# fverdoja/Fast-3D-Pointcloud-Segmentation

Measured on AMD Instinct MI355X. Metric: Mpoints/sec segmented end-to-end, 1M-pt RGB-D frames, higher is better.
Workload: dtype f32

## Files before the change

### fast-3d-pointcloud-segmentation_amd/csrc/f3ds_hip.hip

```cpp
#include <hip/hip_runtime.h>

#include <algorithm>
#include <cmath>
#include <atomic>
#include <map>
#include <chrono>
#include <cstdio>
#include <cstdlib>
#include <cstring>
#include <string>
#include <type_traits>
#include <mutex>
#include <set>
#include <vector>

#include "../../include/f3ds.h"
#include "f3ds_algo.h"
#include "f3ds_glasbey.h"
#include "f3ds_eval.h"
#include "f3ds_dev.h"
#include "f3ds_levels.h"
#include "f3ds_eval_levels.h"
#include "f3ds_rgbd.h"
#include "f3ds_label_image.h"
// ... 492 lines not shown
    const uint32_t capV = (uint32_t)std::max<uint64_t>(256u, std::min<uint64_t>(fin, dcap));
    c->vox_cap = capV;
    uint64_t *k0, *k1; uint32_t *ploc, *v0, *v1, *part, *vkey, *vcount, *seg_start, *list; uint2* bo_te; float* vf; int* pt_voxel;
    const uint32_t nchunks = (dcap + DS_CHUNK - 1u) / DS_CHUNK;
    ENSURE(c->pslot, n, ploc); ENSURE(c->keys0, dcap, k0); ENSURE(c->keys1, dcap, k1); ENSURE(c->vals0, dcap, v0); ENSURE(c->vals1, dcap, v1);
    { uint32_t* w; ENSURE(c->hcnt, (size_t)ntiles * VT_TAB * 2 + 2u * nchunks, w); bo_te = reinterpret_cast<uint2*>(w); part = w + (size_t)ntiles * VT_TAB * 2; }
    ENSURE(c->vkey, (size_t)capV * 3, vkey); ENSURE(c->vcount, capV, vcount); ENSURE(c->vf, (size_t)capV * 12, vf);
    ENSURE(c->seg_start, (size_t)capV + 1, seg_start); ENSURE(c->vlist, n, list); ENSURE(c->pt_voxel, n, pt_voxel);
    { uint32_t *f, *incl; ENSURE(c->flags, capV, f); ENSURE(c->incl, capV, incl); }
    c->idxbits = -1; c->ks = nullptr; c->vs = nullptr;
    rec<d_tile_keys>(c, std::min<uint32_t>(ntiles, (uint32_t)g_grid_cap * 16u), 0u, c->d_pts, n, c->fa, c->d_grid, ploc, k0, v0, dcap, tile_bits, c->d_dc);
    uint64_t* ks; uint32_t* vs;
    int rc = radix_sort(c, k0, v0, k1, v1, dcap, code_bits + tile_bits, &ks, &vs, VT_CNT_BITS, &c->d_dc->seg_count);
    if (rc) return rc;
    rec<d_desc_part>(c, nchunks, 0u, ks, dcap, tile_bits, part, c->d_dc);
    rec<d_desc_offsets>(c, 1u, 0u, part, dcap, capV, seg_start, c->d_dc);
    rec<d_desc_apply>(c, nchunks, 0u, ks, vs, dcap, capV, tile_bits, c->fa, c->d_grid, part, bo_te, seg_start, vkey, c->d_dc);
    rec<d_tile_place>(c, std::min<uint32_t>(ntiles, (uint32_t)g_grid_cap * 16u), 0u, ploc, n, bo_te, list, pt_voxel, c->d_dc);
    rec<d_voxel_list_accum>(c, std::min<uint32_t>(grid_wide(capV, 256), std::max<uint32_t>(64u, grid_wide(n / 8u, 256))), 0u, c->d_pts, list, seg_start, c->fa, vf, vcount, c->d_dc, capV);
    c->vox_hashed = true;
    return F3DS_OK;
}
int seg_neighbors(f3ds_ctx* c, uint32_t wgs) {
    const uint32_t V = c->V;
    const bool blocks = c->h_dc->depth <= N_BLOCK_DEPTH_MAX;
    const uint32_t cap = blocks ? pow2_ge((size_t)V + 16) : pow2_ge((size_t)V * 2 + 16);
    const size_t words = blocks ? (size_t)cap * 2 : cap;
    uint32_t* hvals = nullptr; int *nbr, *nbrT; uint64_t* hkeys;
    c->hmask = cap - 1;
    ENSURE(c->nbr, (size_t)V * 27, nbr); ENSURE(c->nbrT, (size_t)V * 27, nbrT); ENSURE(c->hkeys, words, hkeys);
    if (!blocks) ENSURE(c->hvals, cap, hvals);
    rec_fill(c, hkeys, 0xFFFFFFFFu, words * 8);
    rec<d_vox_table>(c, wgs, 0u, c->vkey.p, V, c->d_grid, hkeys, hvals, c->hmask);
    rec<d_neighbors>(c, grid_wide((size_t)V * 27, 256), 0u, c->vkey.p, c->d_dc, c->d_grid, c->fa.leaf_order, hkeys, hvals, c->hmask, nbr, nbrT);
    return F3DS_OK;
}
int seg_voxels(f3ds_ctx* c) {
    const uint32_t V = c->V, n = c->n;
    if (c->vox_hashed) return seg_neighbors(c, 1u);
    uint32_t *vkey, *vcount; float *vf;
    ENSURE(c->vkey, (size_t)V * 3, vkey); ENSURE(c->vcount, V, vcount); ENSURE(c->vf, (size_t)V * 12, vf);
    if (g_sw.split_voxel_accum) {
        P16* spts; ENSURE(c->spts, n, spts);
        rec<d_point_gather>(c, grid_wide(n, 256), 0u, c->d_pts, c->vs, c->ks, c->idxbits < 0 ? 0 : c->idxbits, c->incl.p, n, c->d_dc, spts, c->pt_voxel.p);
        rec<d_voxel_accum>(c, grid_wide(V, 256), 0u, spts, c->ks, c->idxbits < 0 ? 0 : c->idxbits, c->seg_start.p, c->d_dc, c->fa, c->d_grid, vkey, vcount, vf);
    } else
        rec<d_voxel_gather_accum>(c, grid_wide(V, 256), 0u, c->d_pts, c->vs, c->ks, c->idxbits < 0 ? 0 : c->idxbits, c->seg_start.p, n, c->d_dc, c->fa, c->d_grid, vkey, vcount, vf, c->pt_voxel.p);
    return seg_neighbors(c, grid_for(V, 4096));
}
int seg_normals(f3ds_ctx* c) {
    const uint32_t nt = (c->V + NT_TILE - 1) / NT_TILE;
    uint32_t *tn1, *tord, *tslots;
    ENSURE(c->tile_n1, nt, tn1); ENSURE(c->tile_ord, (size_t)nt * NT_RING1, tord); ENSURE(c->tile_slots, (size_t)nt * SW_SLOT_WORDS * NT_TILE, tslots);
#ifdef F3DS_NORMALS_LOOP
    static const uint32_t budget = dev_getenv("F3DS_NORMALS_WGS") ? (uint32_t)atoi(dev_getenv("F3DS_NORMALS_WGS")) : 0u;
#else
    static const uint32_t budget = 0u;
#endif
    const uint32_t share = budget ? std::max(2u, budget / (uint32_t)g_batch_frames) : nt;
    const int nthr_env = g_sw.normals_threads;
    const uint32_t holes = g_sw.tile_holes;
    if (nthr_env ? nthr_env == 256 : g_batch_frames >= 16)
        rec<d_normals_t<256>>(c, std::min(nt, share), 0u, c->vf.p, c->nbr.p, c->d_dc, tn1, tord, tslots, holes);
    else
        rec<d_normals_t<384>>(c, std::min(nt, share), 0u, c->vf.p, c->nbr.p, c->d_dc, tn1, tord, tslots, holes);
    return F3DS_OK;
}
// ... 90 lines not shown
        const uint32_t nrounds = rounds ? g_sw.r_rounds : 0u;
        rec<d_sweep_R_first>(c, grid_for(V, 256), 0u, a, a_sweep_tag(t), t, nrounds);
        for (uint32_t r = 1; r < nrounds; ++r) rec<d_sweep_R_round>(c, grid_for(V, 256), 0u, a, t, r, nrounds);
        for (uint32_t pass = 0; pass < F3DS_R_PASSES; ++pass) rec<d_sweep_R>(c, pass == 0 ? grid_for(V, 256) : 64u, 0u, a, a_sweep_tag(t), t, pass);
        rec<d_sweep_R_tail>(c, 1u, 0u, a, a_sweep_tag(t), t);
        rec<d_sweep_claim>(c, grid_for(V, 256), 0u, a, t);
        rec<d_centroid>(c, grid_for((size_t)S0 * 64u, 256), 0u, a, t);
    }
    return F3DS_OK;
}
int seg_sweeps(f3ds_ctx* c) {
    SweepBufs sb{&c->owner0, &c->dist0, &c->hc, &c->hcount, &c->hlo, &c->hhi, &c->ghost_vox, &c->ghost_active, &c->ghost_done, &c->ghost_head, &c->ghost_next, &c->htiles, &c->htcnt, c->vf.p, c->seed_kept.p, false};
    return seg_sweeps_on(c, sb);
}
int seg_supervoxels(f3ds_ctx* c) {
    const uint32_t V = c->V, S0 = c->S0;
    uint32_t *loff, *rcnt0, *ev0, *ev1; float *rows, *racc0, *rrec0; int* row_voxel; unsigned char* ralive0; uint64_t *ehk, *ek0, *ek1;
    ENSURE(c->loff, S0 + 2, loff);
    int rc = scan_u32(c, c->hcount.p, loff + 1, S0 + 1);
    if (rc) return rc;
    rec_fill(c, loff, 0u, 4);
    ENSURE(c->rows, ((size_t)V + S0 + 1) * 12, rows); ENSURE(c->row_voxel, (size_t)V + S0 + 1, row_voxel);
    ENSURE(c->racc0, (size_t)(S0 + 1) * 12, racc0); ENSURE(c->rcnt0, S0 + 1, rcnt0); ENSURE(c->rrec0, (size_t)(S0 + 1) * 16, rrec0);
    ENSURE(c->ralive0, S0 + 1, ralive0);
    rec_fill(c, ralive0, 0u, S0 + 1);
    rec_fill(c, rcnt0, 0u, (size_t)(S0 + 1) * 4);
    rec<d_sv_fill>(c, S0 ? (S0 + 3u) / 4u : 1u, 0u,
                   c->vf.p, c->owner0.p, S0, c->hlo.p, c->hhi.p, c->ghost_vox.p, c->ghost_active.p, c->hcount.p, loff, c->hc.p, rows, row_voxel, racc0, rcnt0, rrec0, ralive0, c->d_dc, c->htiles.p, c->htcnt.p, V);
    const uint32_t ecap = (uint32_t)std::min<uint64_t>((uint64_t)S0 * c->edge_mult + 1024u, 0x7fffffffu);
    const uint32_t ehcap = pow2_ge((size_t)ecap * 2);
    ENSURE(c->ehk, ehcap, ehk);
    ENSURE(c->ekeys0, ecap, ek0); ENSURE(c->ekeys1, ecap, ek1); ENSURE(c->evals0, ecap, ev0); ENSURE(c->evals1, ecap, ev1);
    rec_fill(c, ehk, 0xFFFFFFFFu, (size_t)ehcap * 8);
    rec<d_edges>(c, grid_for(V, 256), 0u, V, S0, c->nbrT.p, c->owner0.p, ehk, ehcap - 1, ek0, ecap, c->d_dc);
    rec<d_edges_ghost>(c, grid_for(S0, 256), 0u, V, S0, c->ghost_vox.p, c->ghost_active.p, c->nbrT.p, c->owner0.p, ehk, ehcap - 1, ek0, ecap, c->d_dc);
    return F3DS_OK;
}
int seg_edge_sort(f3ds_ctx* c, int sort_bits) {
    const uint32_t E = c->E, S0 = c->S0;
    uint32_t *ea0, *eb0; ENSURE(c->ea0, E, ea0); ENSURE(c->eb0, E, eb0);
    uint32_t* evs;
    { uint32_t* h; ENSURE(c->hist, (size_t)RS_BINS * (((size_t)E * 2 + RS_TILE - 1) / RS_TILE + 1), h); }
    rec<d_iota>(c, grid_for(E, 256), 0u, c->evals0.p, E);
    int rc = radix_sort(c, c->ekeys0.p, c->evals0.p, c->ekeys1.p, c->evals1.p, E, sort_bits, &c->eks, &evs);
    if (rc) return rc;
    rec<d_edge_init>(c, grid_for(E, 256), 0u, c->eks, E, S0, ea0, eb0);
    return F3DS_OK;
}
bool merge_il_layout(uint32_t E, uint32_t S0, int nw, int res, MergeLds* xl) {
    memset(xl, 0, sizeof *xl);
    if ((uint64_t)E * (res == 2 ? 10u : 2u) > (1u << 22)) return false;
    const MergeIlLayout L = merge_il_offsets(E, nw, res);
    xl->Ecap = L.Ecap; xl->NGcap = L.NGcap; xl->lds_bytes = L.total; xl->keys_in_lds = res;
    xl->spec = g_sw.merge_spec ? 1 : 0;
    return L.total <= MC_LDS_LIMIT && S0 <= 65534u;
}
enum MergeKind { MK_GLOBAL = 0, MK_IL = 1 };
inline int mk_waves(int kind) { return (kind - MK_IL) >= 2 ? 4 : 8; }
inline int mk_res(int kind) { return (kind - MK_IL) % 2 ? 0 : 2; }
int choose_merge_kind(const std::vector<f3ds_ctx*>& fr, bool force_global) {
    if (force_global || g_sw.force_global_merge) return MK_GLOBAL;
    const bool e_keys = g_sw.merge_keys >= 0;
    const bool shared = fr.size() >= 16 && g_batch_calls[fr[0]->device & 15].load(std::memory_order_relaxed) >= 2;
    const int nw = g_sw.merge_nw ? (g_sw.merge_nw == 8 ? 8 : 4) : (shared ? 4 : 8);
    const int first = e_keys ? (g_sw.merge_keys == 2 ? 2 : 0) : (shared ? g_merge_shared_res : 2);
    for (int res = first; res >= (e_keys ? first : 0); res -= 2) {
        bool ok = true;
// ... 1800 lines not shown
```

### fast-3d-pointcloud-segmentation_amd/csrc/f3ds_kernels.inc

```


namespace {

struct P16 { float x, y, z; uint32_t rgba; };

struct DevCounters {
    unsigned long long n_finite;
    uint32_t bbox[6];
    uint32_t bbox_any;
    uint32_t n_valid;
    uint32_t n_voxels;
    uint32_t n_cells;
    uint32_t n_seeds;
    uint32_t n_edges;
    uint32_t n_alive;
    uint32_t n_merges;
    uint32_t n_regions;
    uint32_t n_events;
    int error;
    int r_overflow;
    float lambda;
    uint32_t seg_count;
    uint32_t n_ghosts;
    int depth;
// ... 281 lines not shown
struct __attribute__((aligned(16))) BtEntry { uint32_t key, base; unsigned long long vacant; };
static_assert(sizeof(BtEntry) == 16, "one 16-byte load per probe");
template <class T> __device__ inline bool vt_cas(T* p, T* expect, T v, bool agent) {
    return agent ? __hip_atomic_compare_exchange_strong(p, expect, v, __ATOMIC_RELAXED, __ATOMIC_RELAXED, __HIP_MEMORY_SCOPE_AGENT)
                 : __hip_atomic_compare_exchange_strong(p, expect, v, __ATOMIC_RELAXED, __ATOMIC_RELAXED, __HIP_MEMORY_SCOPE_WORKGROUP);
}
__device__ inline void vt_insert(uint64_t* hkeys, uint32_t* hvals, uint32_t hmask, bool agent, unsigned x, unsigned y, unsigned z, uint32_t v) {
    const unsigned long long pk = (unsigned long long)n_pack_key(x, y, z);
    uint32_t h = (uint32_t)hash64((uint64_t)pk) & hmask;
    for (;;) {
        unsigned long long expect = HASH_EMPTY;
        if (vt_cas((unsigned long long*)&hkeys[h], &expect, pk, agent) || expect == pk) { hvals[h] = v; return; }
        h = (h + 1u) & hmask;
    }
}
__device__ inline int vt_find(const uint64_t* hkeys, const uint32_t* hvals, uint32_t hmask, unsigned x, unsigned y, unsigned z) {
    const uint64_t pk = n_pack_key(x, y, z);
    uint32_t h = (uint32_t)hash64(pk) & hmask;
    for (;;) {
        const uint64_t k = hkeys[h];
        if (k == pk) return (int)hvals[h];
        if (k == HASH_EMPTY) return -1;
        h = (h + 1u) & hmask;
    }
}
__device__ inline BtEntry* bt_entry(BtEntry* tab, uint32_t tmask, bool agent, uint32_t bk) {
    uint32_t h = (uint32_t)hash64((uint64_t)bk) & tmask;
    for (;;) {
        uint32_t expect = BT_EMPTY;
        if (vt_cas(&tab[h].key, &expect, bk, agent) || expect == bk) return &tab[h];
        h = (h + 1u) & tmask;
    }
}
__device__ inline int bt_find(const BtEntry* tab, uint32_t tmask, int leaf_order, unsigned x, unsigned y, unsigned z) {
    const uint32_t bk = n_block_key(x, y, z);
    uint32_t h = (uint32_t)hash64((uint64_t)bk) & tmask;
    for (;;) {
        const uint4 e = reinterpret_cast<const uint4*>(tab)[h];
        if (e.x == bk) return n_block_ordinal(e.y, ~(((uint64_t)e.w << 32) | (uint64_t)e.z), n_block_cell(x, y, z), leaf_order);
        if (e.x == BT_EMPTY) return -1;
        h = (h + 1u) & tmask;
    }
}
struct RgbdArgs {
    uint32_t width, n;
    uint32_t depth_pitch, color_pitch;
    int depth_f32, color_format;
    float depth_scale, fx, fy, cx, cy;
};
template <class T> __device__ inline T load_unaligned(const unsigned char* p) { T t; __builtin_memcpy(&t, p, sizeof(T)); return t; }
template <bool DEPTH_F32, int COLOR>
__device__ inline void deproject_loop(const unsigned char* depth, const unsigned char* color, const RgbdArgs& a, P16* out) {
    const uint32_t stride = gridDim.x * blockDim.x;
    const uint32_t sv = stride / a.width, su = stride - sv * a.width;
    uint32_t i = BIX * blockDim.x + threadIdx.x;
    uint32_t v = i / a.width, u = i - v * a.width;
    for (; i < a.n; i += stride) {
        const unsigned char* drow = depth + (size_t)v * a.depth_pitch;
        const unsigned char* crow = color + (size_t)v * a.color_pitch;
        float z = 0.0f;
        bool valid;
        if constexpr (DEPTH_F32) valid = n_depth_to_z(reinterpret_cast<const float*>(drow)[u], a.depth_scale, z);
        else valid = n_depth_to_z(reinterpret_cast<const uint16_t*>(drow)[u], a.depth_scale, z);
        uint32_t rgba;
        if constexpr (COLOR == 0) { const unsigned char* p = crow + 3u * (size_t)u; rgba = n_color_word(p[0], p[1], p[2], 255u); }
        else {
            const uint32_t w = load_unaligned<uint32_t>(crow + 4u * (size_t)u);
            rgba = COLOR == 1 ? n_color_word(w & 255u, (w >> 8) & 255u, (w >> 16) & 255u, w >> 24) : w;
        }
        float x, y, zo;
        n_deproject(u, v, valid, z, a.fx, a.fy, a.cx, a.cy, x, y, zo);
        reinterpret_cast<uint4*>(out)[i] = make_uint4(__float_as_uint(x), __float_as_uint(y), __float_as_uint(zo), rgba);
        u += su; v += sv;
        if (u >= a.width) { u -= a.width; ++v; }
    }
}
// ... 607 lines not shown
                for (uint32_t j = 0; j < VG_CHUNK / 256; ++j) buf[j * 256u + tid] = q[j];
                __syncthreads();
                const uint32_t a = s > c0 ? s : c0, b = e < c1 ? e : c1;
                for (uint32_t i = a; i < b; ++i) {
                    const uint4 w = buf[i - c0];
                    float z = __uint_as_float(w.z); n_prelude(z, fa.fold_negative_z);
                    sx += __uint_as_float(w.x); sy += __uint_as_float(w.y); sz += z;
                    sr += (float)((w.w >> 16) & 255u); sg += (float)((w.w >> 8) & 255u); sb += (float)(w.w & 255u);
                }
                __syncthreads();
            }
            if (!mine) continue;
            const float c = (float)(e - s);
            vcount[v] = e - s;
            float4* row = reinterpret_cast<float4*>(vf + (size_t)v * 12);
            row[0] = make_float4(sx / c, sy / c, sz / c, sr / c);
            row[1] = make_float4(sg / c, sb / c, 0.0f, 0.0f);
            row[2] = make_float4(0.0f, 0.0f, 0.0f, 0.0f);
        }
    }
};
__device__ inline int hash_find(const uint64_t* hkeys, const uint32_t* hvals, uint32_t hmask, uint64_t pk) {
    uint32_t h = (uint32_t)hash64(pk) & hmask;
    for (;;) {
        uint64_t k = hkeys[h];
        if (k == pk) return (int)hvals[h];
        if (k == HASH_EMPTY) return -1;
        h = (h + 1u) & hmask;
    }
}

struct d_neighbors {
    static constexpr int BLOCK = 256;
    __device__ void operator()(const uint32_t* vkey, const DevCounters* dc, const GridInfo* gp, int leaf_order, const uint64_t* hkeys,
                                                  const uint32_t* hvals, uint32_t hmask, int* nbr, int* nbrT) const {
        __shared__ int tr[27][65];
        const uint32_t V = dc->n_voxels;
        const unsigned max_key = gp->max_key;
        const bool blocks = vt_blocks(gp->depth);
        const BtEntry* const tab = reinterpret_cast<const BtEntry*>(hkeys);
        for (uint32_t vb = BIX * 64u; vb < V; vb += gridDim.x * 64u) {
            const uint32_t nv = V - vb < 64u ? V - vb : 64u, np = nv * 27u;
            for (uint32_t tl = threadIdx.x; tl < np; tl += 256u) {
                const uint32_t vl = tl / 27u, s = tl - vl * 27u, v = vb + vl;
                const int d[3] = {(int)(s / 9u) - 1, (int)((s / 3u) % 3u) - 1, (int)(s % 3u) - 1};
                bool ok = true; unsigned k[3];
                for (int a = 0; a < 3; ++a) {
                    long long q = (long long)vkey[v * 3 + a] + d[a];
                    if (q < 0 || q > (long long)max_key) ok = false;
                    k[a] = (unsigned)q;
                }
                const int u = !ok ? -1 : blocks ? bt_find(tab, hmask, leaf_order, k[0], k[1], k[2]) : vt_find(hkeys, hvals, hmask, k[0], k[1], k[2]);
                nbr[(size_t)vb * 27u + tl] = u;
                tr[s][vl] = u;
            }
            __syncthreads();
            for (uint32_t r = threadIdx.x; r < 27u * 64u; r += 256u) {
                const uint32_t s = r >> 6, vl = r & 63u;
                if (vl < nv) nbrT[(size_t)s * V + vb + vl] = tr[s][vl];
            }
            __syncthreads();
        }
    }
};
constexpr int NT_TILE = 128;
constexpr int NT_HCAP = 2048;
#ifndef F3DS_NT_SLOTS
#define F3DS_NT_SLOTS 896
#endif
#ifndef F3DS_NT_RING1
#define F3DS_NT_RING1 448
#endif
constexpr int NT_SLOTS = F3DS_NT_SLOTS;
constexpr int NT_RING1 = F3DS_NT_RING1;
constexpr uint16_t NT_NONE = 0xFFFFu;
constexpr uint32_t NT_HNONE = 0x3FFu;
constexpr uint32_t NT_ORD_LIMIT = (1u << 22) - 2u;
static_assert(NT_SLOTS < 1023, "slot numbers share a word with the ordinal");
constexpr uint16_t NT_ZERO = NT_SLOTS;
constexpr uint32_t SW_TILE_NONE = 0xFFFFFFFFu;
constexpr int SW_SLOT_BITS = 9;
constexpr int SW_SLOT_WORDS = (27 * SW_SLOT_BITS + 31) / 32;
static_assert(NT_RING1 < (1 << SW_SLOT_BITS), "a list position must fit its bit field");
__device__ __forceinline__ void sw_slots_pack(const uint32_t pos[27], uint32_t w[SW_SLOT_WORDS]) {
#pragma unroll
// ... 784 lines not shown
#pragma unroll
    for (int k0 = 0; k0 < 27; k0 += 9) {
        int nu[9];
#pragma unroll
        for (int k = 0; k < 9; ++k) nu[k] = ROWS ? a_nbr_w(s, v, k0 + k) : a_nbr(s, v, k0 + k);
#pragma unroll
        for (int k = 0; k < 9; ++k) {
            const int u = nu[k] >= 0 ? nu[k] : v;
            a[u >> 6] = stamp; b[u >> 6] = stamp;
        }
    }
}
struct d_sweep_begin {
    static constexpr bool LATENCY_KERNEL = true;
    static constexpr int BLOCK = 256;
    __device__ void operator()(SweepFrame f, uint32_t t) const {
        __shared__ uint32_t s_n;
        if (threadIdx.x == 0) s_n = 0;
        for (uint32_t h = 1 + threadIdx.x; h <= f.S0; h += blockDim.x) if (f.ghost_vox[h] >= 0) f.ghost_head[f.ghost_vox[h]] = 0u;
        __syncthreads();
        uint32_t mine = 0;
        for (uint32_t h = 1 + threadIdx.x; h <= f.S0; h += blockDim.x)
            if (f.ghost_active[h]) { f.ghost_next[h] = atomicExch(&f.ghost_head[f.ghost_vox[h]], h); mine++; }
        if (mine) atomicAdd(&s_n, mine);
        __syncthreads();
        if (threadIdx.x == 0) {
            f.dc->n_ghosts = s_n;
            if (t == 0u) f.dc->sweep_stats[0] = f.dc->sweep_stats[1] = f.dc->sweep_stats[2] = f.dc->sweep_stats[3] = 0u;
            if (!a_sweep_begin(sweep_ctl(f.dc), t, s_n, f.thr)) { f.dc->sweep_stats[F3DS_SWEEP_IDLE]++; return; }
            for (int p = 0; p <= F3DS_R_PASSES; ++p) f.dc->rq[p] = 0u;
        }
    }
};
struct SweepTile {
    uint32_t (*lds)[NT_RING1 + 1];
    uint32_t (*lds2)[NT_RING1 + 1];
    int half, li;
    static constexpr int SR = (NT_RING1 + NT_TILE - 1) / NT_TILE;
    __device__ bool stage(const SweepFrame& f, uint32_t tl, const uint32_t* src, const uint32_t* src2) {
        uint32_t n1 = SW_TILE_NONE;
        if (f.tile_n1 && tl * (uint32_t)NT_TILE < (uint32_t)f.sv.V) n1 = f.tile_n1[tl];
        const bool tiled = n1 != SW_TILE_NONE;
        uint32_t a[SR], b[SR];
        if (tiled) {
            const uint32_t* ord = f.tile_ord + (size_t)tl * NT_RING1;
            uint32_t u[SR];
#pragma unroll
            for (int k = 0; k < SR; ++k) { const uint32_t i = (uint32_t)(li + k * NT_TILE); u[k] = ord[i < n1 ? i : 0u]; }
#pragma unroll
            for (int k = 0; k < SR; ++k) a[k] = src[u[k]];
            if (src2) {
#pragma unroll
                for (int k = 0; k < SR; ++k) b[k] = src2[u[k]];
            }
        }
        __syncthreads();
        if (tiled) {
#pragma unroll
            for (int k = 0; k < SR; ++k) { const uint32_t i = (uint32_t)(li + k * NT_TILE); if (i < n1) { lds[half][i] = a[k]; if (src2) lds2[half][i] = b[k]; } }
            if (li == 0) { lds[half][NT_RING1] = 0u; lds2[half][NT_RING1] = 0u; }
        }
        __syncthreads();
        return tiled;
    }
    __device__ bool stage_held(const SweepFrame& f, uint32_t tl) {
        uint32_t n1 = SW_TILE_NONE;
        if (f.tile_n1 && tl * (uint32_t)NT_TILE < (uint32_t)f.sv.V) n1 = f.tile_n1[tl];
        const bool tiled = n1 != SW_TILE_NONE;
        uint32_t g[SR], r[SR];
        if (tiled) {
            const uint32_t* ord = f.tile_ord + (size_t)tl * NT_RING1;
            uint32_t u[SR];
#pragma unroll
            for (int k = 0; k < SR; ++k) { const uint32_t i = (uint32_t)(li + k * NT_TILE); u[k] = ord[i < n1 ? i : 0u]; }
#pragma unroll
            for (int k = 0; k < SR; ++k) { g[k] = f.sv.owner[u[k]]; r[k] = f.ownR[u[k]]; }
        }
        __syncthreads();
        if (tiled) {
#pragma unroll
            for (int k = 0; k < SR; ++k) { const uint32_t i = (uint32_t)(li + k * NT_TILE); if (i < n1) lds[half][i] = (r[k] & F3DS_OWNR_RTRUE) ? g[k] : 0u; }
            if (li == 0) lds[half][NT_RING1] = 0u;
        }
        __syncthreads();
        return tiled;
    }
    __device__ void gather(const SweepFrame& f, uint32_t tl, uint32_t out[27], bool* near2) const {
        uint32_t w[SW_SLOT_WORDS];
        const uint32_t* sp = f.tile_slots + (size_t)tl * SW_SLOT_WORDS * NT_TILE + li;
#pragma unroll
        for (int k = 0; k < SW_SLOT_WORDS; ++k) w[k] = sp[k * NT_TILE];
#pragma unroll
        for (int k = 0; k < 27; ++k) out[k] = lds[half][sw_slot(w, k)];
        if (near2) {
            uint32_t any = 0u;
#pragma unroll
            for (int k = 0; k < 27; ++k) any |= lds2[half][sw_slot(w, k)];
            *near2 = any != 0u;
        }
    }
};
__device__ inline uint64_t marked_pairs(const uint32_t* stamps, uint32_t stamp, uint32_t tp0, uint32_t step, uint32_t V, uint32_t* s_marked) {
    const uint32_t k = threadIdx.x >> 2, q = threadIdx.x & 3u;
    const uint32_t v0 = (tp0 + k * step) * 256u + q * 64u;
    const bool on = v0 < V && stamps[v0 >> 6] == stamp;
    const uint64_t b = __ballot(on);
    uint32_t m16 = 0;
    for (int i = 0; i < 16; ++i) m16 |= ((uint32_t)(b >> (4 * i)) & 0xFu) ? 1u << i : 0u;
    __syncthreads();
    if (threadIdx.x < 2) s_marked[threadIdx.x] = 0u;
    __syncthreads();
    if (lane_id() == 0) atomicOr(&s_marked[threadIdx.x >> 7], m16 << (16u * ((threadIdx.x >> 6) & 1u)));
    __syncthreads();
    return (uint64_t)s_marked[0] | ((uint64_t)s_marked[1] << 32);
}
struct d_sweep_R_pre {
    static constexpr int BLOCK = 256;
    __device__ void operator()(SweepFrame f, unsigned char tag, uint32_t t) const {
        if (!a_sweep_is_full(sweep_ctl(f.dc), t)) return;
        __shared__ uint32_t nown[2][NT_RING1 + 1], ngh[2][NT_RING1 + 1];
// ... 743 lines not shown
        if (lane < 12) racc0[(size_t)h * 12 + lane] = acc;
        const float mr = __shfl(acc, 9, 64), mg = __shfl(acc, 10, 64), mb = __shfl(acc, 11, 64);
        float lab[3];
        lab_three_lanes(lane == 0 ? mr : (lane == 1 ? mg : mb), lane, lab);
        if (lane == 0) {
            rcnt0[h] = len; ralive0[h] = 1;
            atomicAdd(&dc->n_alive, 1u);
            float rec[16];
            rec[0] = cxyz[(size_t)i * 3]; rec[1] = cxyz[(size_t)i * 3 + 1]; rec[2] = cxyz[(size_t)i * 3 + 2];
            rec[3] = cnrm[(size_t)i * 3]; rec[4] = cnrm[(size_t)i * 3 + 1]; rec[5] = cnrm[(size_t)i * 3 + 2];
            rec[6] = mr; rec[7] = mg; rec[8] = mb;
            rec[9] = lab[0]; rec[10] = lab[1]; rec[11] = lab[2];
            rec[12] = rec[13] = rec[14] = rec[15] = 0.0f;
            for (int k = 0; k < 16; ++k) rrec0[(size_t)h * 16 + k] = rec[k];
            float* c12 = hc + (size_t)h * 12;
            c12[0] = rec[0]; c12[1] = rec[1]; c12[2] = rec[2]; c12[3] = mr; c12[4] = mg; c12[5] = mb; c12[6] = rec[3]; c12[7] = rec[4]; c12[8] = rec[5]; c12[9] = c12[10] = c12[11] = 0.0f;
        }
    }
};
__device__ inline void edge_insert(uint64_t key, uint64_t* hkeys, uint32_t hmask, uint64_t* ekeys, uint32_t ecap, DevCounters* dc) {
    uint32_t hh = (uint32_t)hash64(key) & hmask;
    for (uint32_t probes = 0; probes <= hmask; ++probes) {
        unsigned long long old = atomicCAS((unsigned long long*)&hkeys[hh], (unsigned long long)HASH_EMPTY, (unsigned long long)key);
        if (old == key) return;
        if (old == HASH_EMPTY) {
            uint32_t pos = atomicAdd(&dc->n_edges, 1u);
            if (pos < ecap) ekeys[pos] = key; else { dc->error = F3DS_ERR_UNSUPPORTED; dc->ev_overflow = 3; }
            return;
        }
        hh = (hh + 1u) & hmask;
    }
    dc->error = F3DS_ERR_UNSUPPORTED;
}
__device__ inline void leaf_edges(uint32_t h, uint32_t v, uint32_t V, uint32_t S0, const int* nbrT, const uint32_t* owner, uint64_t* hkeys, uint32_t hmask,
                                  uint64_t* ekeys, uint32_t ecap, DevCounters* dc) {
    int nu[27]; uint32_t og[27];
#pragma unroll
    for (int s = 0; s < 27; ++s) nu[s] = nbrT[(size_t)s * V + v];
#pragma unroll
    for (int s = 0; s < 27; ++s) {
        const uint32_t o = owner[nu[s] >= 0 ? (uint32_t)nu[s] : v];
        og[s] = (nu[s] >= 0 && o && o != h && h < o) ? o : 0u;
    }
    uint32_t last = 0;
#pragma unroll
    for (int s = 0; s < 27; ++s) {
        const uint32_t o = og[s];
        if (o && o != last) { last = o; edge_insert((uint64_t)h * (S0 + 1ull) + o, hkeys, hmask, ekeys, ecap, dc); }
    }
}
struct d_edges {
    static constexpr int BLOCK = 256;
    __device__ void operator()(uint32_t V, uint32_t S0, const int* nbrT, const uint32_t* owner, uint64_t* hkeys, uint32_t hmask,
                                              uint64_t* ekeys, uint32_t ecap, DevCounters* dc) const {
        for (uint32_t v = BIX * blockDim.x + threadIdx.x; v < V; v += gridDim.x * blockDim.x) {
            const uint32_t h = owner[v];
            if (h) leaf_edges(h, v, V, S0, nbrT, owner, hkeys, hmask, ekeys, ecap, dc);
        }
    }
};
struct d_edges_ghost {
    static constexpr int BLOCK = 256;
    __device__ void operator()(uint32_t V, uint32_t S0, const int* ghost_vox, const unsigned char* ghost_active, const int* nbrT,
                                                    const uint32_t* owner, uint64_t* hkeys, uint32_t hmask, uint64_t* ekeys, uint32_t ecap, DevCounters* dc) const {
        for (uint32_t h = 1 + BIX * blockDim.x + threadIdx.x; h <= S0; h += gridDim.x * blockDim.x)
            if (ghost_active[h]) leaf_edges(h, (uint32_t)ghost_vox[h], V, S0, nbrT, owner, hkeys, hmask, ekeys, ecap, dc);
    }
};
struct d_iota {
    static constexpr int BLOCK = 256;
    __device__ void operator()(uint32_t* v, uint32_t n) const {
        for (uint32_t i = BIX * blockDim.x + threadIdx.x; i < n; i += gridDim.x * blockDim.x) v[i] = i;
    }
};
struct d_fill_f32 {
    static constexpr int BLOCK = 256;
    __device__ void operator()(float* v, uint32_t n, float x) const {
        for (uint32_t i = BIX * blockDim.x + threadIdx.x; i < n; i += gridDim.x * blockDim.x) v[i] = x;
    }
};
struct d_edge_init {
    static constexpr int BLOCK = 256;
    __device__ void operator()(const uint64_t* ekeys, uint32_t E, uint32_t S0, uint32_t* ea0, uint32_t* eb0) const {
        for (uint32_t e = BIX * blockDim.x + threadIdx.x; e < E; e += gridDim.x * blockDim.x) {
            ea0[e] = (uint32_t)(ekeys[e] / (S0 + 1ull)); eb0[e] = (uint32_t)(ekeys[e] % (S0 + 1ull));
        }
    }
};
struct d_edge_deltas {
    static constexpr int BLOCK = 256;
// ... 1300 lines not shown
```

### fast-3d-pointcloud-segmentation_amd/csrc/f3ds_numerics.h

```cpp
#ifndef F3DS_NUMERICS_H_
#define F3DS_NUMERICS_H_

#include "f3ds_math.h"

namespace f3ds {

#define F3DS_FLT_MAX 3.402823466e+38f
#define F3DS_FLT_MIN 1.175494351e-38f
#define F3DS_FLT_EPS 1.192092896e-07f

F3DS_HD float n_sqrtf(float x) { return __builtin_sqrtf(x); }
F3DS_HD double n_sqrt(double x) { return __builtin_sqrt(x); }
F3DS_HD bool n_finite3(float x, float y, float z) { return m_isfinitef(x) && m_isfinitef(y) && m_isfinitef(z); }
F3DS_HD float n_nanf() { return m_from_bitsf(0x7fc00000u); }

struct GridInfo {
    double min[3];
    double max[3];
    double res;
    int depth;
    unsigned max_key;
    int error;
    int empty;
};
// ... 77 lines not shown
}
F3DS_HD uint64_t n_spread3_21(uint64_t v) {
    v = (v | (v << 32)) & 0x001F00000000FFFFull;
    v = (v | (v << 16)) & 0x001F0000FF0000FFull;
    v = (v | (v << 8)) & 0x100F00F00F00F00Full;
    v = (v | (v << 4)) & 0x10C30C30C30C30C3ull;
    v = (v | (v << 2)) & 0x1249249249249249ull;
    return v;
}
F3DS_HD uint64_t n_morton(unsigned x, unsigned y, unsigned z, int depth) {
    if (depth <= 10) {
        const uint32_t m = (1u << depth) - 1u;
        return (uint64_t)((n_spread3_10(x & m) << 2) | (n_spread3_10(y & m) << 1) | n_spread3_10(z & m));
    }
    const uint64_t m = (1ull << depth) - 1ull;
    return (n_spread3_21(x & m) << 2) | (n_spread3_21(y & m) << 1) | n_spread3_21(z & m);
}
F3DS_HD void n_demorton(uint64_t c, int depth, unsigned key[3]) {
    unsigned x = 0, y = 0, z = 0;
    for (int b = depth - 1; b >= 0; --b) {
        unsigned d = (unsigned)(c >> (3 * b)) & 7u;
        x = (x << 1) | ((d >> 2) & 1u);
        y = (y << 1) | ((d >> 1) & 1u);
        z = (z << 1) | (d & 1u);
    }
    key[0] = x; key[1] = y; key[2] = z;
}
F3DS_HD uint64_t n_pack_key(unsigned x, unsigned y, unsigned z) {
    return ((uint64_t)x << 42) | ((uint64_t)y << 21) | (uint64_t)z;
}
#define N_BLOCK_DEPTH_MAX 12
F3DS_HD uint32_t n_block_key(unsigned x, unsigned y, unsigned z) { return ((x >> 2) << 20) | ((y >> 2) << 10) | (z >> 2); }
F3DS_HD unsigned n_block_cell(unsigned x, unsigned y, unsigned z) { return (unsigned)n_morton(x & 3u, y & 3u, z & 3u, 2); }
F3DS_HD int n_block_ordinal(uint32_t base, uint64_t mask, unsigned cell, int leaf_order) {
    if (!((mask >> cell) & 1ull)) return -1;
    const uint64_t before = leaf_order == 1 ? ((mask >> cell) >> 1) : (mask & ((1ull << cell) - 1ull));
    return (int)(base + (uint32_t)__builtin_popcountll(before));
}

F3DS_HD void n_roots2(float b, float c, float r[3]) {
    r[0] = 0.0f;
    float d = (float)((double)(b * b) - 4.0 * (double)c);
    if (d < 0.0f) d = 0.0f;
    float sd = n_sqrtf(d);
    r[2] = 0.5f * (b + sd);
    r[1] = 0.5f * (b - sd);
}
template <class K = m_lit> F3DS_HD void n_roots(float m00, float m01, float m02, float m11, float m12, float m22, float r[3], K mc = K()) {
    float c0 = m00 * m11 * m22 + 2.0f * m01 * m02 * m12 - m00 * m12 * m12 - m11 * m02 * m02 - m22 * m01 * m01;
    float c1 = m00 * m11 - m01 * m01 + m00 * m22 - m02 * m02 + m11 * m22 - m12 * m12;
    float c2 = m00 + m11 + m22;
    if (m_absf(c0) < F3DS_FLT_EPS) { n_roots2(c2, c1, r); return; }
    const float inv3 = (float)(1.0 / 3.0);
    const float sqrt3 = 1.7320508075688772f;
    float c2_3 = c2 * inv3;
    float a_3 = (c1 - c2 * c2_3) * inv3;
    if (a_3 > 0.0f) a_3 = 0.0f;
    float half_b = 0.5f * (c0 + c2_3 * (2.0f * c2_3 * c2_3 - c1));
    float q = half_b * half_b + a_3 * a_3 * a_3;
    if (q > 0.0f) q = 0.0f;
    float rho = n_sqrtf(-a_3);
    float theta = m_atan2f(n_sqrtf(-q), half_b, mc) * inv3;
    float ct = m_cosf(theta, mc), st = m_sinf(theta, mc);
    r[0] = c2_3 + 2.0f * rho * ct;
    r[1] = c2_3 - rho * (ct + sqrt3 * st);
    r[2] = c2_3 - rho * (ct - sqrt3 * st);
    float t;
    if (r[0] >= r[1]) { t = r[0]; r[0] = r[1]; r[1] = t; }
    if (r[1] >= r[2]) {
        t = r[1]; r[1] = r[2]; r[2] = t;
// ... 188 lines not shown
```

Measured before the change: 3750.

## Resolve voxel neighbors per voxel via 8 block lookups and tile edge owners

In block-hash mode, the neighbor kernel now handles one voxel per thread instead of one of its 27 slots. Each thread probes only the up to 8 adjacent 4x4x4 blocks in parallel, derives all 27 ordinals from the block occupancy masks, and transposes the results through per-wave LDS for coalesced nbr writes. This replaces 27 independent hash probes per voxel. The edge kernel now reuses the sweep tile staging to gather neighbor owners from LDS tiles when tile data is available, falling back to nbrT reads otherwise. This adds register pressure and more complex control flow in exchange.

```diff
diff --git a/fast-3d-pointcloud-segmentation_amd/csrc/f3ds_hip.hip b/fast-3d-pointcloud-segmentation_amd/csrc/f3ds_hip.hip
--- a/fast-3d-pointcloud-segmentation_amd/csrc/f3ds_hip.hip
+++ b/fast-3d-pointcloud-segmentation_amd/csrc/f3ds_hip.hip
@@ -548,7 +548,7 @@
     if (!blocks) ENSURE(c->hvals, cap, hvals);
     rec_fill(c, hkeys, 0xFFFFFFFFu, words * 8);
     rec<d_vox_table>(c, wgs, 0u, c->vkey.p, V, c->d_grid, hkeys, hvals, c->hmask);
-    rec<d_neighbors>(c, grid_wide((size_t)V * 27, 256), 0u, c->vkey.p, c->d_dc, c->d_grid, c->fa.leaf_order, hkeys, hvals, c->hmask, nbr, nbrT);
+    rec<d_neighbors>(c, grid_wide(blocks ? (size_t)V : (size_t)V * 27, 256), 0u, c->vkey.p, c->d_dc, c->d_grid, c->fa.leaf_order, hkeys, hvals, c->hmask, nbr, nbrT);
     return F3DS_OK;
 }
 int seg_voxels(f3ds_ctx* c) {
@@ -705,7 +705,8 @@
     ENSURE(c->ehk, ehcap, ehk);
     ENSURE(c->ekeys0, ecap, ek0); ENSURE(c->ekeys1, ecap, ek1); ENSURE(c->evals0, ecap, ev0); ENSURE(c->evals1, ecap, ev1);
     rec_fill(c, ehk, 0xFFFFFFFFu, (size_t)ehcap * 8);
-    rec<d_edges>(c, grid_for(V, 256), 0u, V, S0, c->nbrT.p, c->owner0.p, ehk, ehcap - 1, ek0, ecap, c->d_dc);
+    const TileView tiles{g_sw.sweep_tiles ? c->tile_n1.p : nullptr, c->tile_ord.p, c->tile_slots.p, V};
+    rec<d_edges>(c, grid_for(V, 256), 0u, tiles, S0, c->nbrT.p, c->owner0.p, ehk, ehcap - 1, ek0, ecap, c->d_dc);
     rec<d_edges_ghost>(c, grid_for(S0, 256), 0u, V, S0, c->ghost_vox.p, c->ghost_active.p, c->nbrT.p, c->owner0.p, ehk, ehcap - 1, ek0, ecap, c->d_dc);
     return F3DS_OK;
 }
diff --git a/fast-3d-pointcloud-segmentation_amd/csrc/f3ds_kernels.inc b/fast-3d-pointcloud-segmentation_amd/csrc/f3ds_kernels.inc
--- a/fast-3d-pointcloud-segmentation_amd/csrc/f3ds_kernels.inc
+++ b/fast-3d-pointcloud-segmentation_amd/csrc/f3ds_kernels.inc
@@ -337,16 +337,6 @@
         h = (h + 1u) & tmask;
     }
 }
-__device__ inline int bt_find(const BtEntry* tab, uint32_t tmask, int leaf_order, unsigned x, unsigned y, unsigned z) {
-    const uint32_t bk = n_block_key(x, y, z);
-    uint32_t h = (uint32_t)hash64((uint64_t)bk) & tmask;
-    for (;;) {
-        const uint4 e = reinterpret_cast<const uint4*>(tab)[h];
-        if (e.x == bk) return n_block_ordinal(e.y, ~(((uint64_t)e.w << 32) | (uint64_t)e.z), n_block_cell(x, y, z), leaf_order);
-        if (e.x == BT_EMPTY) return -1;
-        h = (h + 1u) & tmask;
-    }
-}
 struct RgbdArgs {
     uint32_t width, n;
     uint32_t depth_pitch, color_pitch;
@@ -1020,13 +1010,74 @@
 
 struct d_neighbors {
     static constexpr int BLOCK = 256;
+    static constexpr int TILE_WORDS = 64 * 27;
+    template <class T> __device__ static __forceinline__ T pick(int j, T c0, T c1, T c2, T c3, T c4, T c5, T c6, T c7) {
+        const bool cx = j & 4, cy = j & 2, cz = j & 1;
+        const T z0 = cz ? c1 : c0, z1 = cz ? c3 : c2, z2 = cz ? c5 : c4, z3 = cz ? c7 : c6;
+        const T y0 = cy ? z1 : z0, y1 = cy ? z3 : z2;
+        return cx ? y1 : y0;
+    }
+    template <class T> __device__ static __forceinline__ T pick(int j, const T (&c)[8]) { return pick(j, c[0], c[1], c[2], c[3], c[4], c[5], c[6], c[7]); }
+    template <int S> __device__ static __forceinline__ int ordinal(const NVoxelBlocks& b, const uint32_t (&base)[8], const uint64_t (&occ)[8], const unsigned (&cell)[3][3], int leaf_order) {
+        const int j = n_voxel_slot_block(b, S);
+        if (j < 0) return -1;
+        return n_block_ordinal(pick(j, base), pick(j, occ), cell[0][S / 9] | cell[1][(S / 3) % 3] | cell[2][S % 3], leaf_order);
+    }
+    template <int S0> __device__ static __forceinline__ void ordinals9(const NVoxelBlocks& b, const uint32_t (&base)[8], const uint64_t (&occ)[8], const unsigned (&cell)[3][3], int leaf_order, int (&u)[27]) {
+        u[S0] = ordinal<S0>(b, base, occ, cell, leaf_order); u[S0 + 1] = ordinal<S0 + 1>(b, base, occ, cell, leaf_order); u[S0 + 2] = ordinal<S0 + 2>(b, base, occ, cell, leaf_order);
+        u[S0 + 3] = ordinal<S0 + 3>(b, base, occ, cell, leaf_order); u[S0 + 4] = ordinal<S0 + 4>(b, base, occ, cell, leaf_order); u[S0 + 5] = ordinal<S0 + 5>(b, base, occ, cell, leaf_order);
+        u[S0 + 6] = ordinal<S0 + 6>(b, base, occ, cell, leaf_order); u[S0 + 7] = ordinal<S0 + 7>(b, base, occ, cell, leaf_order); u[S0 + 8] = ordinal<S0 + 8>(b, base, occ, cell, leaf_order);
+    }
+    __device__ static void per_voxel(int* lds, const uint32_t* vkey, uint32_t V, unsigned max_key, int leaf_order, const uint4* tab, uint32_t tmask, int* nbr, int* nbrT) {
+        const uint32_t w = threadIdx.x >> 6, lane = threadIdx.x & 63u;
+        int* const tile = lds + w * (uint32_t)TILE_WORDS;
+        for (uint32_t vb = (BIX * 4u + w) * 64u; vb < V; vb += gridDim.x * 256u) {
+            const uint32_t nv = V - vb < 64u ? V - vb : 64u;
+            const uint32_t v = vb + (lane < nv ? lane : nv - 1u);
+            const unsigned k[3] = {vkey[v * 3], vkey[v * 3 + 1], vkey[v * 3 + 2]};
+            const NVoxelBlocks b = n_voxel_blocks(k[0], k[1], k[2], max_key);
+            uint32_t h[8]; uint4 e[8];
+#pragma unroll
+            for (int j = 0; j < 8; ++j) h[j] = (uint32_t)hash64((uint64_t)b.key[j]) & tmask;
+#pragma unroll
+            for (int j = 0; j < 8; ++j) e[j] = tab[h[j]];
+            for (uint32_t step = 0; step < tmask; ++step) {
+                bool again = false;
+#pragma unroll
+                for (int j = 0; j < 8; ++j)
+                    if (e[j].x != b.key[j] && e[j].x != BT_EMPTY) { h[j] = (h[j] + 1u) & tmask; e[j] = tab[h[j]]; again = true; }
+                if (!again) break;
+            }
+            uint32_t base[8]; uint64_t occ[8];
+#pragma unroll
+            for (int j = 0; j < 8; ++j) { base[j] = e[j].y; occ[j] = e[j].x == b.key[j] ? ~(((uint64_t)e[j].w << 32) | (uint64_t)e[j].z) : 0ull; }
+            unsigned cell[3][3];
+#pragma unroll
+            for (int a = 0; a < 3; ++a)
+#pragma unroll
+                for (int d = 0; d < 3; ++d) cell[a][d] = n_block_cell_axis(k[a] + (unsigned)d - 1u, a);
+            int u[27];
+            ordinals9<0>(b, base, occ, cell, leaf_order, u); ordinals9<9>(b, base, occ, cell, leaf_order, u); ordinals9<18>(b, base, occ, cell, leaf_order, u);
+            if (lane < nv) {
+#pragma unroll
+                for (int s = 0; s < 27; ++s) nbrT[(size_t)s * V + v] = u[s];
+            }
+#pragma unroll
+            for (int s = 0; s < 27; ++s) tile[lane * 27u + (uint32_t)s] = u[s];
+            wave_lds_sync();
+#pragma unroll
+            for (int i = 0; i < 27; ++i) { const uint32_t r = (uint32_t)i * 64u + lane; if (r < nv * 27u) nbr[(size_t)vb * 27u + r] = tile[r]; }
+            wave_lds_sync();
+        }
+    }
     __device__ void operator()(const uint32_t* vkey, const DevCounters* dc, const GridInfo* gp, int leaf_order, const uint64_t* hkeys,
                                                   const uint32_t* hvals, uint32_t hmask, int* nbr, int* nbrT) const {
-        __shared__ int tr[27][65];
+        __shared__ int lds[4 * TILE_WORDS];
         const uint32_t V = dc->n_voxels;
         const unsigned max_key = gp->max_key;
-        const bool blocks = vt_blocks(gp->depth);
-        const BtEntry* const tab = reinterpret_cast<const BtEntry*>(hkeys);
+        if (vt_blocks(gp->depth)) { per_voxel(lds, vkey, V, max_key, leaf_order, reinterpret_cast<const uint4*>(hkeys), hmask, nbr, nbrT); return; }
+        int (*const tr)[65] = reinterpret_cast<int (*)[65]>(lds);
+        static_assert(27 * 65 <= 4 * TILE_WORDS, "the per-slot path's tile fits");
         for (uint32_t vb = BIX * 64u; vb < V; vb += gridDim.x * 64u) {
             const uint32_t nv = V - vb < 64u ? V - vb : 64u, np = nv * 27u;
             for (uint32_t tl = threadIdx.x; tl < np; tl += 256u) {
@@ -1038,7 +1089,7 @@
                     if (q < 0 || q > (long long)max_key) ok = false;
                     k[a] = (unsigned)q;
                 }
-                const int u = !ok ? -1 : blocks ? bt_find(tab, hmask, leaf_order, k[0], k[1], k[2]) : vt_find(hkeys, hvals, hmask, k[0], k[1], k[2]);
+                const int u = !ok ? -1 : vt_find(hkeys, hvals, hmask, k[0], k[1], k[2]);
                 nbr[(size_t)vb * 27u + tl] = u;
                 tr[s][vl] = u;
             }
@@ -1889,14 +1940,20 @@
         }
     }
 };
+struct TileView {
+    const uint32_t *tile_n1, *tile_ord, *tile_slots;
+    uint32_t V;
+};
+__device__ __forceinline__ uint32_t tile_view_V(const SweepFrame& f) { return (uint32_t)f.sv.V; }
+__device__ __forceinline__ uint32_t tile_view_V(const TileView& f) { return f.V; }
 struct SweepTile {
     uint32_t (*lds)[NT_RING1 + 1];
     uint32_t (*lds2)[NT_RING1 + 1];
     int half, li;
     static constexpr int SR = (NT_RING1 + NT_TILE - 1) / NT_TILE;
-    __device__ bool stage(const SweepFrame& f, uint32_t tl, const uint32_t* src, const uint32_t* src2) {
+    template <class F> __device__ bool stage(const F& f, uint32_t tl, const uint32_t* src, const uint32_t* src2) {
         uint32_t n1 = SW_TILE_NONE;
-        if (f.tile_n1 && tl * (uint32_t)NT_TILE < (uint32_t)f.sv.V) n1 = f.tile_n1[tl];
+        if (f.tile_n1 && tl * (uint32_t)NT_TILE < tile_view_V(f)) n1 = f.tile_n1[tl];
         const bool tiled = n1 != SW_TILE_NONE;
         uint32_t a[SR], b[SR];
         if (tiled) {
@@ -1942,7 +1999,7 @@
         __syncthreads();
         return tiled;
     }
-    __device__ void gather(const SweepFrame& f, uint32_t tl, uint32_t out[27], bool* near2) const {
+    template <class F> __device__ void gather(const F& f, uint32_t tl, uint32_t out[27], bool* near2) const {
         uint32_t w[SW_SLOT_WORDS];
         const uint32_t* sp = f.tile_slots + (size_t)tl * SW_SLOT_WORDS * NT_TILE + li;
 #pragma unroll
@@ -2752,30 +2809,46 @@
     }
     dc->error = F3DS_ERR_UNSUPPORTED;
 }
+__device__ inline void owner_edges(uint32_t h, const uint32_t on[27], uint32_t S0, uint64_t* hkeys, uint32_t hmask, uint64_t* ekeys, uint32_t ecap, DevCounters* dc) {
+    uint32_t last = 0;
+#pragma unroll
+    for (int s = 0; s < 27; ++s) {
+        const uint32_t o = (on[s] && on[s] != h && h < on[s]) ? on[s] : 0u;
+        if (o && o != last) { last = o; edge_insert((uint64_t)h * (S0 + 1ull) + o, hkeys, hmask, ekeys, ecap, dc); }
+    }
+}
+__device__ __forceinline__ void leaf_owners(uint32_t v, uint32_t V, const int* nbrT, const uint32_t* owner, uint32_t og[27]) {
+    int nu[27];
+#pragma unroll
+    for (int s = 0; s < 27; ++s) nu[s] = nbrT[(size_t)s * V + v];
+#pragma unroll
+    for (int s = 0; s < 27; ++s) {
+        const uint32_t o = owner[nu[s] >= 0 ? (uint32_t)nu[s] : v];
+        og[s] = nu[s] >= 0 ? o : 0u;
+    }
+}
 __device__ inline void leaf_edges(uint32_t h, uint32_t v, uint32_t V, uint32_t S0, const int* nbrT, const uint32_t* owner, uint64_t* hkeys, uint32_t hmask,
                                   uint64_t* ekeys, uint32_t ecap, DevCounters* dc) {
-    int nu[27]; uint32_t og[27];
-#pragma unroll
-    for (int s = 0; s < 27; ++s) nu[s] = nbrT[(size_t)s * V + v];
-#pragma unroll
-    for (int s = 0; s < 27; ++s) {
-        const uint32_t o = owner[nu[s] >= 0 ? (uint32_t)nu[s] : v];
-        og[s] = (nu[s] >= 0 && o && o != h && h < o) ? o : 0u;
-    }
-    uint32_t last = 0;
-#pragma unroll
-    for (int s = 0; s < 27; ++s) {
-        const uint32_t o = og[s];
-        if (o && o != last) { last = o; edge_insert((uint64_t)h * (S0 + 1ull) + o, hkeys, hmask, ekeys, ecap, dc); }
-    }
+    uint32_t og[27];
+    leaf_owners(v, V, nbrT, owner, og);
+    owner_edges(h, og, S0, hkeys, hmask, ekeys, ecap, dc);
 }
 struct d_edges {
     static constexpr int BLOCK = 256;
-    __device__ void operator()(uint32_t V, uint32_t S0, const int* nbrT, const uint32_t* owner, uint64_t* hkeys, uint32_t hmask,
+    __device__ void operator()(TileView t, uint32_t S0, const int* nbrT, const uint32_t* owner, uint64_t* hkeys, uint32_t hmask,
                                               uint64_t* ekeys, uint32_t ecap, DevCounters* dc) const {
-        for (uint32_t v = BIX * blockDim.x + threadIdx.x; v < V; v += gridDim.x * blockDim.x) {
-            const uint32_t h = owner[v];
-            if (h) leaf_edges(h, v, V, S0, nbrT, owner, hkeys, hmask, ekeys, ecap, dc);
+        __shared__ uint32_t nown[2][NT_RING1 + 1];
+        const uint32_t V = t.V;
+        SweepTile st{nown, nown, (int)(threadIdx.x >> 7), (int)(threadIdx.x & 127u)};
+        for (uint32_t tp = BIX; tp * 256u < V; tp += gridDim.x) {
+            const uint32_t tl = tp * 2u + (uint32_t)st.half;
+            const uint32_t v = tl * (uint32_t)NT_TILE + (uint32_t)st.li;
+            const bool tiled = st.stage(t, tl, owner, nullptr);
+            const uint32_t h = v < V ? owner[v] : 0u;
+            if (!h) continue;
+            uint32_t og[27];
+            if (tiled) st.gather(t, tl, og, nullptr); else leaf_owners(v, V, nbrT, owner, og);
+            owner_edges(h, og, S0, hkeys, hmask, ekeys, ecap, dc);
         }
     }
 };
diff --git a/fast-3d-pointcloud-segmentation_amd/csrc/f3ds_numerics.h b/fast-3d-pointcloud-segmentation_amd/csrc/f3ds_numerics.h
--- a/fast-3d-pointcloud-segmentation_amd/csrc/f3ds_numerics.h
+++ b/fast-3d-pointcloud-segmentation_amd/csrc/f3ds_numerics.h
@@ -133,10 +133,41 @@
 #define N_BLOCK_DEPTH_MAX 12
 F3DS_HD uint32_t n_block_key(unsigned x, unsigned y, unsigned z) { return ((x >> 2) << 20) | ((y >> 2) << 10) | (z >> 2); }
 F3DS_HD unsigned n_block_cell(unsigned x, unsigned y, unsigned z) { return (unsigned)n_morton(x & 3u, y & 3u, z & 3u, 2); }
+F3DS_HD unsigned n_block_cell_axis(unsigned q, int a) { return (((q & 2u) << 2) | (q & 1u)) << (2 - a); }
 F3DS_HD int n_block_ordinal(uint32_t base, uint64_t mask, unsigned cell, int leaf_order) {
     if (!((mask >> cell) & 1ull)) return -1;
     const uint64_t before = leaf_order == 1 ? ((mask >> cell) >> 1) : (mask & ((1ull << cell) - 1ull));
     return (int)(base + (uint32_t)__builtin_popcountll(before));
+}
+struct NVoxelBlocks {
+    uint32_t key[8];
+    unsigned need;
+    unsigned cross[3], out[3];
+};
+F3DS_HD uint32_t n_block_axis(unsigned k, unsigned max_key, unsigned* cross, unsigned* out) {
+    uint32_t other = k >> 2;
+    unsigned c = 0u, o = 0u;
+    if (k == 0u) o |= 1u; else if ((k & 3u) == 0u) { c |= 1u; other = (k >> 2) - 1u; }
+    if (k >= max_key) o |= 4u; else if ((k & 3u) == 3u) { c |= 4u; other = (k >> 2) + 1u; }
+    *cross = c; *out = o;
+    return other;
+}
+F3DS_HD NVoxelBlocks n_voxel_blocks(unsigned x, unsigned y, unsigned z, unsigned max_key) {
+    NVoxelBlocks b;
+    const uint32_t x0 = (x >> 2) << 20, x1 = n_block_axis(x, max_key, &b.cross[0], &b.out[0]) << 20;
+    const uint32_t y0 = (y >> 2) << 10, y1 = n_block_axis(y, max_key, &b.cross[1], &b.out[1]) << 10;
+    const uint32_t z0 = z >> 2, z1 = n_block_axis(z, max_key, &b.cross[2], &b.out[2]);
+    b.key[0] = x0 | y0 | z0; b.key[1] = x0 | y0 | z1; b.key[2] = x0 | y1 | z0; b.key[3] = x0 | y1 | z1;
+    b.key[4] = x1 | y0 | z0; b.key[5] = x1 | y0 | z1; b.key[6] = x1 | y1 | z0; b.key[7] = x1 | y1 | z1;
+    const unsigned other = (b.cross[0] ? 4u : 0u) | (b.cross[1] ? 2u : 0u) | (b.cross[2] ? 1u : 0u);
+    b.need = 0u;
+    for (unsigned j = 0; j < 8u; ++j) if ((j & ~other) == 0u) b.need |= 1u << j;
+    return b;
+}
+F3DS_HD int n_voxel_slot_block(const NVoxelBlocks& b, int s) {
+    const unsigned mx = 1u << (s / 9), my = 1u << ((s / 3) % 3), mz = 1u << (s % 3);
+    if ((b.out[0] & mx) || (b.out[1] & my) || (b.out[2] & mz)) return -1;
+    return (int)(((b.cross[0] & mx) ? 4u : 0u) | ((b.cross[1] & my) ? 2u : 0u) | ((b.cross[2] & mz) ? 1u : 0u));
 }
 
 F3DS_HD void n_roots2(float b, float c, float r[3]) {
```

Result: no change. 3745 (-0.1%).
